# castorini/daam

Measured on NVIDIA H100. Metric: heatmap px/s (layers x steps x tokens), higher is better.
Workload: dtype bf16

## Files before the change

daam_b200/csrc/accumulate_mma.cu:

```cuda
#include <cuda.h>

#include <mutex>
#include <type_traits>
#include <unordered_map>
#include <string>

#include "common.cuh"

namespace daam {
namespace {

constexpr int kStages = 2;
constexpr int kAccStages = 3;
constexpr int kPrefetchTiles = 6;
constexpr int kQBytes = kTilePixels * 128;
constexpr int kKBytes = kTokensPad * 128;
constexpr int kStageBytes = kQBytes + kKBytes;
constexpr int kPBytes = kTokens * kTilePixels * 4;
constexpr int kConsumers = 256;
constexpr int kThreads = kConsumers + 32;
constexpr int kThreads16 = kConsumers + 64;
constexpr int kBarBytes = 64;
constexpr int kBarBytes16 = 8 * 2 * (kStages + kAccStages);
constexpr int kSmemBytes = 1024 + kStages * kStageBytes + kAccStages * kPBytes + kBarBytes16;
constexpr int kSlabSmemBytes = kSmemBytes + kPBytes;
constexpr int kSplitStageBytes = 2 * kStageBytes;
constexpr int kSplitSmemBytes = 1024 + (kStages + 1) * kSplitStageBytes + kPBytes + kBarBytes;
static_assert(kSmemBytes <= 232448, "16-bit form exceeds the 227 KB shared-memory limit");
static_assert(kSplitSmemBytes <= 232448, "split form exceeds the 227 KB shared-memory limit");
static_assert(kSlabSmemBytes <= 232448, "16-bit second-slab form exceeds the 227 KB shared-memory limit");
constexpr int long_smem_bytes(int chunks) {
  return 1024 + kStages * (kQBytes + chunks * kKBytes) + kAccStages * kPBytes + kBarBytes16;
}
static_assert(long_smem_bytes(3) <= 232448, "16-bit long-context form exceeds the 227 KB shared-memory limit");

struct MmaParams {
  LaunchParams base;
  CUtensorMap qmap[kMaxLayersPerLaunch];
  CUtensorMap kmap[kMaxLayersPerLaunch];
  CUtensorMap amap[kMaxLayersPerLaunch];
};
struct MmaSlabParams : MmaParams {
  CUtensorMap smap[kMaxLayersPerLaunch];
  float* slab[kMaxLayersPerLaunch];
};
template <bool kSecond>
using MmaParamsT = std::conditional_t<kSecond, MmaSlabParams, MmaParams>;

__device__ __forceinline__ uint32_t smem_u32(const void* p) { return (uint32_t)__cvta_generic_to_shared(p); }

__device__ __forceinline__ void mbar_init(uint32_t bar, uint32_t count) {
  asm volatile("mbarrier.init.shared::cta.b64 [%0], %1;" ::"r"(bar), "r"(count));
}
__device__ __forceinline__ void mbar_arrive(uint32_t bar) {
  asm volatile("mbarrier.arrive.shared::cta.b64 _, [%0];" ::"r"(bar) : "memory");
}
__device__ __forceinline__ void mbar_expect_tx(uint32_t bar, uint32_t bytes) {
  asm volatile("mbarrier.arrive.expect_tx.shared::cta.b64 _, [%0], %1;" ::"r"(bar), "r"(bytes) : "memory");
}
__device__ __forceinline__ bool mbar_try(uint32_t bar, uint32_t parity) {
  uint32_t ok;
  asm volatile(
      "{\n"
      ".reg .pred p;\n"
      "mbarrier.try_wait.parity.shared::cta.b64 p, [%1], %2;\n"
      "selp.u32 %0, 1, 0, p;\n"
      "}"
      : "=r"(ok)
      : "r"(bar), "r"(parity)
      : "memory");
  return ok != 0;
}
#ifndef DAAM_MBAR_TIMEOUT_CYCLES
#define DAAM_MBAR_TIMEOUT_CYCLES 20000000000LL
#endif
__device__ __forceinline__ void mbar_wait(uint32_t bar, uint32_t parity) {
  if (mbar_try(bar, parity)) return;
#if DAAM_MBAR_TIMEOUT_CYCLES > 0
  const long long t0 = clock64();
  while (!mbar_try(bar, parity)) {
    if (clock64() - t0 > DAAM_MBAR_TIMEOUT_CYCLES) __trap();
  }
#else
  while (!mbar_try(bar, parity)) {}
#endif
}

__device__ __forceinline__ void tma_load_4d(const CUtensorMap* map, uint32_t bar, uint32_t dst, int c0, int c1, int c2,
                                            int c3) {
  asm volatile(
      "cp.async.bulk.tensor.4d.shared::cluster.global.mbarrier::complete_tx::bytes [%0], [%1, {%3, %4, %5, %6}], [%2];"
      ::"r"(dst), "l"(reinterpret_cast<uint64_t>(map)), "r"(bar), "r"(c0), "r"(c1), "r"(c2), "r"(c3)
      : "memory");
}
__device__ __forceinline__ void tma_store_2d(const CUtensorMap* map, uint32_t src, int c0, int c1) {
  asm volatile("cp.async.bulk.tensor.2d.global.shared::cta.bulk_group [%0, {%2, %3}], [%1];" ::"l"(
                   reinterpret_cast<uint64_t>(map)),
               "r"(src), "r"(c0), "r"(c1)
               : "memory");
}
__device__ __forceinline__ void tma_reduce_add_2d(const CUtensorMap* map, uint32_t src, int c0, int c1) {
  asm volatile("cp.reduce.async.bulk.tensor.2d.global.shared::cta.add.tile.bulk_group [%0, {%2, %3}], [%1];" ::"l"(
                   reinterpret_cast<uint64_t>(map)),
               "r"(src), "r"(c0), "r"(c1)
               : "memory");
}
__device__ __forceinline__ uint64_t l2_evict_last() {
  uint64_t p;
  asm volatile("createpolicy.fractional.L2::evict_last.b64 %0, 1.0;" : "=l"(p));
  return p;
}
__device__ __forceinline__ uint64_t l2_evict_first() {
  uint64_t p;
  asm volatile("createpolicy.fractional.L2::evict_first.b64 %0, 1.0;" : "=l"(p));
  return p;
}
__device__ __forceinline__ void tma_prefetch_4d(const CUtensorMap* map, int c0, int c1, int c2, int c3, uint64_t pol) {
  asm volatile("cp.async.bulk.prefetch.tensor.4d.L2.global.tile.L2::cache_hint [%0, {%1, %2, %3, %4}], %5;"
               ::"l"(reinterpret_cast<uint64_t>(map)), "r"(c0), "r"(c1), "r"(c2), "r"(c3), "l"(pol)
               : "memory");
}
__device__ __forceinline__ void tma_load_2d_hint(const CUtensorMap* map, uint32_t bar, uint32_t dst, int c0, int c1,
                                                 uint64_t pol) {
  asm volatile(
      "cp.async.bulk.tensor.2d.shared::cluster.global.mbarrier::complete_tx::bytes.L2::cache_hint [%0], [%1, {%3, %4}], "
      "[%2], %5;"
      ::"r"(dst), "l"(reinterpret_cast<uint64_t>(map)), "r"(bar), "r"(c0), "r"(c1), "l"(pol)
      : "memory");
}
__device__ __forceinline__ void tma_store_2d_hint(const CUtensorMap* map, uint32_t src, int c0, int c1, uint64_t pol) {
  asm volatile("cp.async.bulk.tensor.2d.global.shared::cta.bulk_group.L2::cache_hint [%0, {%2, %3}], [%1], %4;" ::"l"(
                   reinterpret_cast<uint64_t>(map)),
               "r"(src), "r"(c0), "r"(c1), "l"(pol)
               : "memory");
}
__device__ __forceinline__ void prefetch_tensormap(const CUtensorMap* map) {
  asm volatile("prefetch.tensormap [%0];" ::"l"(reinterpret_cast<uint64_t>(map)) : "memory");
}
__device__ __forceinline__ void bulk_commit() { asm volatile("cp.async.bulk.commit_group;" ::: "memory"); }
__device__ __forceinline__ void bulk_wait_read0() { asm volatile("cp.async.bulk.wait_group.read 0;" ::: "memory"); }
__device__ __forceinline__ void bulk_wait_read1() { asm volatile("cp.async.bulk.wait_group.read 1;" ::: "memory"); }
__device__ __forceinline__ void fence_proxy_async() { asm volatile("fence.proxy.async.shared::cta;" ::: "memory"); }
__device__ __forceinline__ void consumer_barrier() { asm volatile("bar.sync 1, %0;" ::"n"(kConsumers) : "memory"); }

__device__ __forceinline__ uint64_t wgmma_desc_sw128(uint32_t smem_addr) {
  return (uint64_t)((smem_addr & 0x3FFFFu) >> 4) | (1ull << 16)  |
         ((uint64_t)(1024 >> 4) << 32)  | (1ull << 62) ;
}

using Frag = float[40];

__device__ __forceinline__ void frag_fence(Frag& d) {
#pragma unroll
  for (int i = 0; i < 40; ++i) asm volatile("" : "+f"(d[i])::"memory");
}
__device__ __forceinline__ void wgmma_fence() { asm volatile("wgmma.fence.sync.aligned;" ::: "memory"); }
__device__ __forceinline__ void wgmma_commit() { asm volatile("wgmma.commit_group.sync.aligned;" ::: "memory"); }
__device__ __forceinline__ void wgmma_wait0() { asm volatile("wgmma.wait_group.sync.aligned 0;" ::: "memory"); }

#define DAAM_FRAG_OPERANDS                                                                                          \
  "+f"(d[0]), "+f"(d[1]), "+f"(d[2]), "+f"(d[3]), "+f"(d[4]), "+f"(d[5]), "+f"(d[6]), "+f"(d[7]), "+f"(d[8]),         \
      "+f"(d[9]), "+f"(d[10]), "+f"(d[11]), "+f"(d[12]), "+f"(d[13]), "+f"(d[14]), "+f"(d[15]), "+f"(d[16]),          \
      "+f"(d[17]), "+f"(d[18]), "+f"(d[19]), "+f"(d[20]), "+f"(d[21]), "+f"(d[22]), "+f"(d[23]), "+f"(d[24]),         \
      "+f"(d[25]), "+f"(d[26]), "+f"(d[27]), "+f"(d[28]), "+f"(d[29]), "+f"(d[30]), "+f"(d[31]), "+f"(d[32]),         \
      "+f"(d[33]), "+f"(d[34]), "+f"(d[35]), "+f"(d[36]), "+f"(d[37]), "+f"(d[38]), "+f"(d[39])
#define DAAM_FRAG_REGS                                                                                              \
  "{%0, %1, %2, %3, %4, %5, %6, %7, %8, %9, %10, %11, %12, %13, %14, %15, %16, %17, %18, %19, %20, %21, %22, %23, " \
  "%24, %25, %26, %27, %28, %29, %30, %31, %32, %33, %34, %35, %36, %37, %38, %39}"

template <bool kBf16>
__device__ __forceinline__ void wgmma_16bit(Frag& d, uint64_t adesc, uint64_t bdesc) {
  if constexpr (kBf16)
    asm volatile("wgmma.mma_async.sync.aligned.m64n80k16.f32.bf16.bf16 " DAAM_FRAG_REGS ", %40, %41, 1, 1, 1, 0, 0;"
                 : DAAM_FRAG_OPERANDS
                 : "l"(adesc), "l"(bdesc)
                 : "memory");
  else
    asm volatile("wgmma.mma_async.sync.aligned.m64n80k16.f32.f16.f16 " DAAM_FRAG_REGS ", %40, %41, 1, 1, 1, 0, 0;"
                 : DAAM_FRAG_OPERANDS
                 : "l"(adesc), "l"(bdesc)
                 : "memory");
}
__device__ __forceinline__ void wgmma_tf32(Frag& d, uint64_t adesc, uint64_t bdesc) {
  asm volatile("wgmma.mma_async.sync.aligned.m64n80k8.f32.tf32.tf32 " DAAM_FRAG_REGS ", %40, %41, 1, 1, 1;"
               : DAAM_FRAG_OPERANDS
               : "l"(adesc), "l"(bdesc)
               : "memory");
}

struct Tile {
  int li, prompt, head, pixel0;
};
__device__ __forceinline__ Tile decode_tile(const LaunchParams& P, int tile, int& li) {
  while (li + 1 < P.n_layers && tile >= P.layer[li + 1].tile_begin) ++li;
  const LayerParams& L = P.layer[li];
  const int local = tile - L.tile_begin;
  const int ptile = local % L.tiles_per_head;
  const int ph = local / L.tiles_per_head;
  Tile t;
  t.li = li;
  t.head = ph % L.heads;
  t.prompt = ph / L.heads;
  t.pixel0 = ptile * kTilePixels;
  return t;
}

__device__ __forceinline__ int tile_at_weight(const LaunchParams& P, long long w) {
  if (w >= P.total_weight) return P.total_tiles;
  int li = 0;
  while (li + 1 < P.n_layers && w >= P.layer[li + 1].weight_begin) ++li;
  const LayerParams& L = P.layer[li];
  return L.tile_begin + (int)((w - L.weight_begin + L.weight - 1) / L.weight);
}

__device__ __forceinline__ float rna_tf32(float x) {
  uint32_t r;
  asm("cvt.rna.tf32.f32 %0, %1;" : "=r"(r) : "f"(x));
  return __uint_as_float(r);
}
__device__ __forceinline__ float trunc_tf32(float x) { return __uint_as_float(__float_as_uint(x) & 0xffffe000u); }

__device__ __forceinline__ void split_region(uint8_t* raw, uint8_t* lo, int begin, int end, int ctid, int n_conv) {
  const int stride = n_conv * 16;
  for (int off = begin + ctid * 16; off < end; off += 4 * stride) {
    float4 x[4];
#pragma unroll
    for (int u = 0; u < 4; ++u)
      if (off + u * stride < end) x[u] = *reinterpret_cast<const float4*>(raw + off + u * stride);
#pragma unroll
    for (int u = 0; u < 4; ++u)
      if (off + u * stride < end) {
        float4 h, l;
        h.x = trunc_tf32(x[u].x); h.y = trunc_tf32(x[u].y); h.z = trunc_tf32(x[u].z); h.w = trunc_tf32(x[u].w);
        l.x = rna_tf32(x[u].x - h.x); l.y = rna_tf32(x[u].y - h.y);
        l.z = rna_tf32(x[u].z - h.z); l.w = rna_tf32(x[u].w - h.w);
        *reinterpret_cast<float4*>(raw + off + u * stride) = h;
        *reinterpret_cast<float4*>(lo + off + u * stride) = l;
      }
  }
}

template <bool kBf16>
__device__ __forceinline__ void wgmma_chunk_16bit(Frag& d, uint32_t a_src, uint32_t k_src) {
  wgmma_fence();
#pragma unroll
  for (int k = 0; k < 4; ++k) wgmma_16bit<kBf16>(d, wgmma_desc_sw128(a_src + 32 * k), wgmma_desc_sw128(k_src + 32 * k));
  wgmma_commit();
  wgmma_wait0();
}
template <bool kBf16, int kC>
__device__ __forceinline__ void wgmma_chunk_16bit_long(Frag (&d)[kC], uint32_t a_src, uint32_t k_src) {
  wgmma_fence();
#pragma unroll
  for (int c = 0; c < kC; ++c)
#pragma unroll
    for (int k = 0; k < 4; ++k)
      wgmma_16bit<kBf16>(d[c], wgmma_desc_sw128(a_src + 32 * k), wgmma_desc_sw128(k_src + c * kKBytes + 32 * k));
  wgmma_commit();
  wgmma_wait0();
}

__device__ __forceinline__ void griddep_wait() { asm volatile("griddepcontrol.wait;" ::: "memory"); }

template <bool kSplit, bool kChunked, int kSlab, int kC = 1>
__global__ void __launch_bounds__(kSplit ? kThreads : kThreads16, 1)
accumulate_mma_kernel(const __grid_constant__ MmaParamsT<kSlab != kSlabNone> MP) {
  static_assert(kC == 1 || (!kSplit && kSlab == kSlabNone), "long contexts: 16-bit form, plain slab mode only");
  constexpr bool kSecond = kSlab != kSlabNone;
  constexpr int kCtx = kC * kTokens;
  constexpr int kStageBytesT = kSplit ? kSplitStageBytes : kQBytes + kC * kKBytes;
  constexpr int kOperandBytes = (kSplit ? kStages + 1 : kStages) * kStageBytesT;
  constexpr int kPTiles = kSplit ? 1 : kAccStages + (kSecond ? 1 : 0);
  const LaunchParams& P = MP.base;
  extern __shared__ uint8_t smem_raw[];
  const uint32_t raw = smem_u32(smem_raw);
  const uint32_t base = (raw + 1023u) & ~1023u;
  uint8_t* gen = smem_raw + (base - raw);
  float* sP = reinterpret_cast<float*>(gen + kOperandBytes);
  const uint32_t sP_u32 = base + kOperandBytes;
  float* sS = sP + kAccStages * (kTokens * kTilePixels);
  const uint32_t sS_u32 = sP_u32 + kAccStages * kPBytes;
  const uint32_t bars = sP_u32 + kPTiles * kPBytes;
  const uint32_t full0 = bars, empty0 = bars + 8 * kStages;
  const uint32_t afull0 = bars + 16 * kStages, aempty0 = afull0 + 8 * kAccStages;

  const int warp = threadIdx.x >> 5, lane = threadIdx.x & 31;
  int first, count, stride = 1;
  if constexpr (!kChunked && !kSplit) {
    first = blockIdx.x;
    stride = gridDim.x;
    count = (P.total_tiles - (int)blockIdx.x + stride - 1) / stride;
  } else if constexpr (!kChunked) {
    const int per = P.total_tiles / gridDim.x, rem = P.total_tiles % gridDim.x;
    first = blockIdx.x * per + min((int)blockIdx.x, rem);
    count = per + ((int)blockIdx.x < rem ? 1 : 0);
  } else {
    first = tile_at_weight(P, (long long)P.total_weight * blockIdx.x / gridDim.x);
    count = tile_at_weight(P, (long long)P.total_weight * (blockIdx.x + 1) / gridDim.x) - first;
  }

  if (threadIdx.x == 0) {
#pragma unroll
    for (int s = 0; s < kStages; ++s) {
      mbar_init(full0 + 8 * s, 1);
      mbar_init(empty0 + 8 * s, kConsumers / 32);
    }
    if constexpr (!kSplit) {
#pragma unroll
      for (int s = 0; s < kAccStages; ++s) {
        mbar_init(afull0 + 8 * s, 1);
        mbar_init(aempty0 + 8 * s, 1);
      }
    }
    asm volatile("fence.mbarrier_init.release.cluster;" ::: "memory");
  }
  if (count > 0 && lane == 0 && (warp == (kSplit ? 0 : 9) || warp == 8)) {
    int li0 = 0;
    const Tile t0 = decode_tile(P, first, li0);
    if (warp != 8) {
      prefetch_tensormap(&MP.amap[t0.li]);
      if constexpr (kSecond) prefetch_tensormap(&MP.smap[t0.li]);
    } else {
      prefetch_tensormap(&MP.qmap[t0.li]);
      prefetch_tensormap(&MP.kmap[t0.li]);
    }
  }
  __syncthreads();
  if (!P.early_loads) griddep_wait();
  asm volatile("griddepcontrol.launch_dependents;" ::: "memory");

  if (warp == 9) {
    if constexpr (!kSplit) {
      if (lane == 0 && count > 0) {
        if (P.early_loads) griddep_wait();
        const uint64_t pol = l2_evict_first();
        int li = 0;
        for (int i = 0; i < count; ++i) {
          const Tile t = decode_tile(P, first + i * stride, li);
#pragma unroll
          for (int c = 0; c < kC; ++c) {
            const int n = i * kC + c;
            const int a = n % kAccStages;
            mbar_wait(aempty0 + 8 * a, ((uint32_t)(n / kAccStages) & 1u) ^ 1u);
            mbar_expect_tx(afull0 + 8 * a, kPBytes);
            tma_load_2d_hint(&MP.amap[t.li], afull0 + 8 * a, sP_u32 + a * kPBytes, t.pixel0,
                             (t.prompt * P.layer[t.li].heads + t.head) * kCtx + c * kTokens, pol);
          }
        }
      }
    }
  } else if (warp == 8) {
    if (lane == 0) {
      int li = 0, j = 0;
      for (int i = 0; i < count; ++i) {
        if (!kSplit && P.early_loads && i == (kChunked ? 1 : kStages)) {
          const uint64_t pol = l2_evict_last();
          const int end = min(count, i + kPrefetchTiles);
          int pli = 0;
          Tile prev = decode_tile(P, first + (i - 1) * stride, pli);
          for (int p = i; p < end; ++p) {
            const Tile u = decode_tile(P, first + p * stride, pli);
            const bool new_head = u.li != prev.li || u.prompt != prev.prompt || u.head != prev.head;
            const int nc = kChunked ? (P.layer[u.li].head_dim + 63) >> 6 : 1;
            for (int c = 0; c < nc; ++c) {
              tma_prefetch_4d(&MP.qmap[u.li], 64 * c, u.head, u.pixel0, u.prompt, pol);
              if (new_head)
#pragma unroll
                for (int kc = 0; kc < kC; ++kc) tma_prefetch_4d(&MP.kmap[u.li], 64 * c, u.head, kc * kTokens, u.prompt, pol);
            }
            prev = u;
          }
        }
        const Tile t = decode_tile(P, first + i * stride, li);
        const int n_chunks = kChunked ? (P.layer[t.li].head_dim + 63) >> 6 : 1;
        for (int c = 0; c < n_chunks; ++c, ++j) {
          const int s = j % kStages;
          const uint32_t ph = (uint32_t)(j / kStages) & 1u;
          mbar_wait(empty0 + 8 * s, ph ^ 1u);
          const uint32_t q_dst = base + s * kStageBytesT;
          if constexpr (kSplit) {
            const uint32_t k_dst = q_dst + 2 * kQBytes;
            mbar_expect_tx(full0 + 8 * s, kStageBytesT);
            tma_load_4d(&MP.qmap[t.li], full0 + 8 * s, q_dst, 64 * c, t.head, t.pixel0, t.prompt);
            tma_load_4d(&MP.kmap[t.li], full0 + 8 * s, k_dst, 64 * c, t.head, 0, t.prompt);
            tma_load_4d(&MP.qmap[t.li], full0 + 8 * s, q_dst + kQBytes, 64 * c + 32, t.head, t.pixel0, t.prompt);
            tma_load_4d(&MP.kmap[t.li], full0 + 8 * s, k_dst + kKBytes, 64 * c + 32, t.head, 0, t.prompt);
          } else {
            const uint32_t k_dst = q_dst + kQBytes;
            mbar_expect_tx(full0 + 8 * s, kStageBytesT);
            tma_load_4d(&MP.qmap[t.li], full0 + 8 * s, q_dst, 64 * c, t.head, t.pixel0, t.prompt);
#pragma unroll
            for (int kc = 0; kc < kC; ++kc)
              tma_load_4d(&MP.kmap[t.li], full0 + 8 * s, k_dst + kc * kKBytes, 64 * c, t.head, kc * kTokens, t.prompt);
          }
        }
      }
    }
  } else {
    const int tid = threadIdx.x;
    const int wg = warp >> 2;
    const int quad = lane & 3;
    const int r0 = wg * 64 + (warp & 3) * 16 + (lane >> 2);
    int li = 0, j = 0;
    bool issued = false;
    for (int i = 0; i < count; ++i) {
      const Tile t = decode_tile(P, first + i * stride, li);
      const LayerParams& L = P.layer[t.li];
      const int n_chunks = kChunked ? (L.head_dim + 63) >> 6 : 1;
      Frag dd[kC];
      Frag& d = dd[0];
#pragma unroll
      for (int kc = 0; kc < kC; ++kc)
#pragma unroll
        for (int e = 0; e < 40; ++e) dd[kc][e] = 0.f;
      for (int c = 0; c < n_chunks; ++c, ++j) {
        const int s = j % kStages;
        mbar_wait(full0 + 8 * s, (uint32_t)(j / kStages) & 1u);
        const uint32_t q_src = base + s * kStageBytesT;
#pragma unroll
        for (int kc = 0; kc < kC; ++kc) frag_fence(dd[kc]);
        if constexpr (kSplit) {
          uint8_t* stage = gen + s * kStageBytesT;
          uint8_t* lo = gen + kStages * kStageBytesT;
          consumer_barrier();
          split_region(stage, lo, 0, kSplitStageBytes, tid, kConsumers);
          fence_proxy_async();
          consumer_barrier();
          wgmma_fence();
          const uint32_t q_lo = base + kStages * kStageBytesT;
          const uint32_t qa[3] = {q_lo, q_src, q_src};
          const uint32_t kb[3] = {q_src + 2 * kQBytes, q_lo + 2 * kQBytes, q_src + 2 * kQBytes};
#pragma unroll
          for (int p = 0; p < 3; ++p)
#pragma unroll
            for (int k = 0; k < 8; ++k)
              wgmma_tf32(d, wgmma_desc_sw128(qa[p] + (k >> 2) * kQBytes + wg * 64 * 128 + 32 * (k & 3)),
                         wgmma_desc_sw128(kb[p] + (k >> 2) * kKBytes + 32 * (k & 3)));
          wgmma_commit();
          wgmma_wait0();
        } else {
          const uint32_t a_src = q_src + wg * 64 * 128, k_src = q_src + kQBytes;
          if constexpr (kC == 1) {
            if (L.dtype == DAAM_BF16)
              wgmma_chunk_16bit<true>(d, a_src, k_src);
            else
              wgmma_chunk_16bit<false>(d, a_src, k_src);
          } else {
            if (L.dtype == DAAM_BF16)
              wgmma_chunk_16bit_long<true, kC>(dd, a_src, k_src);
            else
              wgmma_chunk_16bit_long<false, kC>(dd, a_src, k_src);
          }
        }
#pragma unroll
        for (int kc = 0; kc < kC; ++kc) frag_fence(dd[kc]);
        __syncwarp();
        if (lane == 0) mbar_arrive(empty0 + 8 * s);
      }

      float m0 = d[0], m1 = d[2];
#pragma unroll
      for (int kc = 0; kc < kC; ++kc)
#pragma unroll
      for (int jj = 0; jj < 10; ++jj) {
        const bool l0 = jj < 9 || quad <= 2, l1 = jj < 9 || quad < 2;
        if (l0) { m0 = fmaxf(m0, dd[kc][4 * jj]); m1 = fmaxf(m1, dd[kc][4 * jj + 2]); }
        if (l1) { m0 = fmaxf(m0, dd[kc][4 * jj + 1]); m1 = fmaxf(m1, dd[kc][4 * jj + 3]); }
      }
      m0 = fmaxf(m0, __shfl_xor_sync(0xffffffffu, m0, 1));
      m0 = fmaxf(m0, __shfl_xor_sync(0xffffffffu, m0, 2));
      m1 = fmaxf(m1, __shfl_xor_sync(0xffffffffu, m1, 1));
      m1 = fmaxf(m1, __shfl_xor_sync(0xffffffffu, m1, 2));
      const float sc = L.scale_log2e, mc0 = m0 * sc, mc1 = m1 * sc;
      float sum0 = 0.f, sum1 = 0.f;
#pragma unroll
      for (int kc = 0; kc < kC; ++kc)
#pragma unroll
      for (int jj = 0; jj < 10; ++jj) {
        const bool l0 = jj < 9 || quad <= 2, l1 = jj < 9 || quad < 2;
        float* f = dd[kc];
        f[4 * jj] = l0 ? fast_exp2(fmaf(f[4 * jj], sc, -mc0)) : 0.f;
        f[4 * jj + 2] = l0 ? fast_exp2(fmaf(f[4 * jj + 2], sc, -mc1)) : 0.f;
        f[4 * jj + 1] = l1 ? fast_exp2(fmaf(f[4 * jj + 1], sc, -mc0)) : 0.f;
        f[4 * jj + 3] = l1 ? fast_exp2(fmaf(f[4 * jj + 3], sc, -mc1)) : 0.f;
        sum0 += f[4 * jj] + f[4 * jj + 1];
        sum1 += f[4 * jj + 2] + f[4 * jj + 3];
      }
      sum0 += __shfl_xor_sync(0xffffffffu, sum0, 1);
      sum0 += __shfl_xor_sync(0xffffffffu, sum0, 2);
      sum1 += __shfl_xor_sync(0xffffffffu, sum1, 1);
      sum1 += __shfl_xor_sync(0xffffffffu, sum1, 2);
      const float inv0 = 1.0f / sum0, inv1 = 1.0f / sum1;

      if constexpr (!kSplit) {
#pragma unroll
        for (int kc = 0; kc < kC; ++kc) {
        const int n = i * kC + kc;
        const int a = n % kAccStages;
        float* sA = sP + a * (kTokens * kTilePixels);
        const bool lowq = quad < 2;
        const int ra = lowq ? r0 : r0 + 8, rb = lowq ? r0 + 8 : r0;
        mbar_wait(afull0 + 8 * a, (uint32_t)(n / kAccStages) & 1u);
        float old[40];
#pragma unroll
        for (int jj = 0; jj < 10; ++jj) {
#pragma unroll
          for (int e = 0; e < 2; ++e) {
            const int col = 8 * jj + 2 * quad + e;
            if (col < kTokens) {
              old[4 * jj + e] = sA[col * kTilePixels + ra];
              old[4 * jj + 2 + e] = sA[col * kTilePixels + rb];
            }
          }
        }
        if constexpr (kSecond) {
          if (tid == 0 && i > 0) bulk_wait_read0();
          consumer_barrier();
        }
        const float* f = dd[kc];
#pragma unroll
        for (int jj = 0; jj < 10; ++jj) {
#pragma unroll
          for (int e = 0; e < 2; ++e) {
            const int col = 8 * jj + 2 * quad + e;
            if (col < kTokens) {
              const float pa = f[4 * jj + e] * inv0, pb = f[4 * jj + 2 + e] * inv1;
              sA[col * kTilePixels + ra] = add_ftz(old[4 * jj + e], lowq ? pa : pb);
              sA[col * kTilePixels + rb] = add_ftz(old[4 * jj + 2 + e], lowq ? pb : pa);
              if constexpr (kSecond) {
                sS[col * kTilePixels + ra] = add_ftz(0.f, lowq ? pa : pb);
                sS[col * kTilePixels + rb] = add_ftz(0.f, lowq ? pb : pa);
              }
            }
          }
        }
        fence_proxy_async();
        consumer_barrier();
        if (tid == 0) {
          tma_store_2d_hint(&MP.amap[t.li], sP_u32 + a * kPBytes, t.pixel0,
                            (t.prompt * L.heads + t.head) * kCtx + kc * kTokens, l2_evict_first());
          if constexpr (kSlab == kSlabStore)
            tma_store_2d(&MP.smap[t.li], sS_u32, t.pixel0, (t.prompt * L.heads + t.head) * kTokens);
          if constexpr (kSlab == kSlabAdd)
            tma_reduce_add_2d(&MP.smap[t.li], sS_u32, t.pixel0, (t.prompt * L.heads + t.head) * kTokens);
          bulk_commit();
          if (n > 0) {
            bulk_wait_read1();
            mbar_arrive(aempty0 + 8 * ((n - 1) % kAccStages));
          }
        }
        }
        continue;
      }

      if (i == 0 && P.early_loads) griddep_wait();

      if (tid == 0 && issued) bulk_wait_read0();
      consumer_barrier();
      const bool lowq = quad < 2;
      const bool stage_ftz = kSlab == kSlabStore && P.rmw_mode == 1;
#pragma unroll
      for (int jj = 0; jj < 10; ++jj) {
#pragma unroll
        for (int e = 0; e < 2; ++e) {
          const int col = 8 * jj + 2 * quad + e;
          if (col < kTokens) {
            float a = d[4 * jj + e] * inv0, b = d[4 * jj + 2 + e] * inv1;
            if constexpr (kSecond) {
              if (stage_ftz) { a = add_ftz(0.f, a); b = add_ftz(0.f, b); }
            }
            sP[col * kTilePixels + (lowq ? r0 : r0 + 8)] = lowq ? a : b;
            sP[col * kTilePixels + (lowq ? r0 + 8 : r0)] = lowq ? b : a;
          }
        }
      }
      if (P.rmw_mode == 1) {
        fence_proxy_async();
        consumer_barrier();
        if (tid == 0) {
          tma_reduce_add_2d(&MP.amap[t.li], sP_u32, t.pixel0, (t.prompt * L.heads + t.head) * kTokens);
          if constexpr (kSlab == kSlabStore)
            tma_store_2d(&MP.smap[t.li], sP_u32, t.pixel0, (t.prompt * L.heads + t.head) * kTokens);
          if constexpr (kSlab == kSlabAdd)
            tma_reduce_add_2d(&MP.smap[t.li], sP_u32, t.pixel0, (t.prompt * L.heads + t.head) * kTokens);
          bulk_commit();
        }
        issued = true;
      } else {
        consumer_barrier();
        const long long hw = L.hw;
        float* acc = L.acc + ((long long)(t.prompt * L.heads + t.head) * kTokens) * hw + t.pixel0;
        const int live = min(kTilePixels, L.hw - t.pixel0) >> 2;
        for (int u = tid; u < kTokens * (kTilePixels / 4); u += kConsumers) {
          const int tok = u / (kTilePixels / 4), c4 = u % (kTilePixels / 4);
          if (c4 < live) {
            float4* g = reinterpret_cast<float4*>(acc + tok * hw) + c4;
            const float4 p = reinterpret_cast<const float4*>(sP + tok * kTilePixels)[c4];
            float4 o = *g;
            o.x += p.x; o.y += p.y; o.z += p.z; o.w += p.w;
            *g = o;
            if constexpr (kSlab == kSlabStore)
              reinterpret_cast<float4*>(MP.slab[t.li] + (acc - L.acc) + tok * hw)[c4] = p;
            if constexpr (kSlab == kSlabAdd) {
              float4* r = reinterpret_cast<float4*>(MP.slab[t.li] + (acc - L.acc) + tok * hw) + c4;
              float4 ro = *r;
              ro.x += p.x; ro.y += p.y; ro.z += p.z; ro.w += p.w;
              *r = ro;
            }
          }
        }
      }
    }
    if (tid == 0 && (kSplit ? issued : count > 0)) bulk_wait_read0();
  }
}

using EncodeFn = CUresult (*)(CUtensorMap*, CUtensorMapDataType, cuuint32_t, void*, const cuuint64_t*,
                              const cuuint64_t*, const cuuint32_t*, const cuuint32_t*, CUtensorMapInterleave,
                              CUtensorMapSwizzle, CUtensorMapL2promotion, CUtensorMapFloatOOBfill);

EncodeFn get_encode() {
  static EncodeFn fn = nullptr;
  static std::once_flag once;
  std::call_once(once, [] {
    void* p = nullptr;
    cudaDriverEntryPointQueryResult q;
    if (cudaGetDriverEntryPoint("cuTensorMapEncodeTiled", &p, cudaEnableDefault, &q) == cudaSuccess &&
        q == cudaDriverEntryPointSuccess)
      fn = reinterpret_cast<EncodeFn>(p);
  });
  return fn;
}

struct MapKey {
  const void* ptr;
  long long s1, s2, s3;
  int d1, d2, d3, kind;
  bool operator==(const MapKey& o) const {
    return ptr == o.ptr && s1 == o.s1 && s2 == o.s2 && s3 == o.s3 && d1 == o.d1 && d2 == o.d2 && d3 == o.d3 &&
           kind == o.kind;
  }
};
struct MapKeyHash {
  size_t operator()(const MapKey& k) const {
    size_t h = reinterpret_cast<size_t>(k.ptr);
    auto mix = [&h](long long v) { h ^= (size_t)v + 0x9e3779b97f4a7c15ull + (h << 6) + (h >> 2); };
    mix(k.s1); mix(k.s2); mix(k.s3); mix(k.d1); mix(k.d2); mix(k.d3); mix(k.kind);
    return h;
  }
};

std::unordered_map<MapKey, CUtensorMap, MapKeyHash>& map_cache() {
  static std::unordered_map<MapKey, CUtensorMap, MapKeyHash> c;
  return c;
}
std::mutex g_map_mu;

int make_qk_map(const void* ptr, int dtype, int head_dim, int heads, int rows, int prompts, long long s_head,
                long long s_row, long long s_prompt, int box_rows, CUtensorMap* out) {
  MapKey key{ptr, s_head, s_row, s_prompt, heads, rows, prompts * 1024 + box_rows, (dtype << 4) | (head_dim << 8)};
  {
    std::lock_guard<std::mutex> lock(g_map_mu);
    auto it = map_cache().find(key);
    if (it != map_cache().end()) { *out = it->second; return DAAM_OK; }
  }
  EncodeFn enc = get_encode();
  if (!enc) { set_error("cuTensorMapEncodeTiled is not available from this driver"); return DAAM_E_CUDA; }
  const cuuint64_t es = dtype == DAAM_F32 ? 4 : 2;
  const cuuint64_t dims[4] = {(cuuint64_t)head_dim, (cuuint64_t)heads, (cuuint64_t)rows, (cuuint64_t)prompts};
  auto bytes = [es](long long s) { return (cuuint64_t)(s > 0 ? s : 8) * es; };
  const cuuint64_t strides[3] = {bytes(s_head), bytes(s_row), bytes(s_prompt)};
  const cuuint32_t box[4] = {(cuuint32_t)(128 / es), 1, (cuuint32_t)box_rows, 1};
  const cuuint32_t estr[4] = {1, 1, 1, 1};
  const CUtensorMapDataType type = dtype == DAAM_F32    ? CU_TENSOR_MAP_DATA_TYPE_FLOAT32
                                   : dtype == DAAM_BF16 ? CU_TENSOR_MAP_DATA_TYPE_BFLOAT16
                                                        : CU_TENSOR_MAP_DATA_TYPE_FLOAT16;
  CUresult r = enc(out, type, 4, const_cast<void*>(ptr), dims, strides, box, estr, CU_TENSOR_MAP_INTERLEAVE_NONE,
                   CU_TENSOR_MAP_SWIZZLE_128B, CU_TENSOR_MAP_L2_PROMOTION_L2_128B, CU_TENSOR_MAP_FLOAT_OOB_FILL_NONE);
  if (r != CUDA_SUCCESS) { set_error("cuTensorMapEncodeTiled(q/k) failed with CUresult %d", (int)r); return DAAM_E_CUDA; }
  std::lock_guard<std::mutex> lock(g_map_mu);
  if (map_cache().size() > 8192) map_cache().clear();
  map_cache()[key] = *out;
  return DAAM_OK;
}

int make_acc_map(float* acc, int hw, int rows, CUtensorMap* out) {
  MapKey key{acc, 0, 0, 0, hw, rows, 0, 1};
  {
    std::lock_guard<std::mutex> lock(g_map_mu);
    auto it = map_cache().find(key);
    if (it != map_cache().end()) { *out = it->second; return DAAM_OK; }
  }
  EncodeFn enc = get_encode();
  if (!enc) { set_error("cuTensorMapEncodeTiled is not available from this driver"); return DAAM_E_CUDA; }
  const cuuint64_t dims[2] = {(cuuint64_t)hw, (cuuint64_t)rows};
  const cuuint64_t strides[1] = {(cuuint64_t)hw * 4};
  const cuuint32_t box[2] = {(cuuint32_t)kTilePixels, (cuuint32_t)kTokens};
  const cuuint32_t estr[2] = {1, 1};
  CUresult r = enc(out, CU_TENSOR_MAP_DATA_TYPE_FLOAT32, 2, acc, dims, strides, box, estr,
                   CU_TENSOR_MAP_INTERLEAVE_NONE, CU_TENSOR_MAP_SWIZZLE_NONE, CU_TENSOR_MAP_L2_PROMOTION_L2_128B,
                   CU_TENSOR_MAP_FLOAT_OOB_FILL_NONE);
  if (r != CUDA_SUCCESS) { set_error("cuTensorMapEncodeTiled(acc) failed with CUresult %d", (int)r); return DAAM_E_CUDA; }
  std::lock_guard<std::mutex> lock(g_map_mu);
  if (map_cache().size() > 8192) map_cache().clear();
  map_cache()[key] = *out;
  return DAAM_OK;
}

struct MmaInstance {
  const void* fn;
  int smem;
};
const MmaInstance kMmaInstances[] = {
    {(const void*)accumulate_mma_kernel<false, false, kSlabNone>, kSmemBytes},
    {(const void*)accumulate_mma_kernel<true, false, kSlabNone>, kSplitSmemBytes},
    {(const void*)accumulate_mma_kernel<false, true, kSlabNone>, kSmemBytes},
    {(const void*)accumulate_mma_kernel<true, true, kSlabNone>, kSplitSmemBytes},
    {(const void*)accumulate_mma_kernel<false, false, kSlabStore>, kSlabSmemBytes},
    {(const void*)accumulate_mma_kernel<true, false, kSlabStore>, kSplitSmemBytes},
    {(const void*)accumulate_mma_kernel<false, true, kSlabStore>, kSlabSmemBytes},
    {(const void*)accumulate_mma_kernel<true, true, kSlabStore>, kSplitSmemBytes},
    {(const void*)accumulate_mma_kernel<false, false, kSlabAdd>, kSlabSmemBytes},
    {(const void*)accumulate_mma_kernel<true, false, kSlabAdd>, kSplitSmemBytes},
    {(const void*)accumulate_mma_kernel<false, true, kSlabAdd>, kSlabSmemBytes},
    {(const void*)accumulate_mma_kernel<true, true, kSlabAdd>, kSplitSmemBytes},
    {(const void*)accumulate_mma_kernel<false, false, kSlabNone, 2>, long_smem_bytes(2)},
    {(const void*)accumulate_mma_kernel<false, true, kSlabNone, 2>, long_smem_bytes(2)},
    {(const void*)accumulate_mma_kernel<false, false, kSlabNone, 3>, long_smem_bytes(3)},
    {(const void*)accumulate_mma_kernel<false, true, kSlabNone, 3>, long_smem_bytes(3)},
};
constexpr int kLongVariant0 = 12;

std::once_flag g_attr_once[64];

}

struct PreparedMma {
  MmaSlabParams mp;
  int grid, block, variant;
  bool second;
};
void* prepared_mma_new() { return new PreparedMma; }
void prepared_mma_delete(void* p) { delete static_cast<PreparedMma*>(p); }

bool mma_supported(const LayerParams& L) {
  const bool prompts_ok = L.n_prompts == 1 || (L.qs_prompt > 0 && L.ks_prompt > 0);
  return L.head_dim % 8 == 0 && L.head_dim <= DAAM_MAX_HEAD_DIM && L.vec_ok && L.qs_head > 0 && L.qs_pixel > 0 &&
         L.ks_head > 0 && L.ks_token > 0 && prompts_ok && L.hw % 4 == 0;
}

int prepare_accumulate_mma(const LaunchParams& p, const SecondSlabs* slabs, SlabMode mode, const DeviceInfo& dev,
                           void* out) {
  if (dev.cc_major != 9) { set_error("the wgmma kernel needs an sm_90 device (found sm_%d%d)", dev.cc_major, dev.cc_minor); return DAAM_E_UNSUPPORTED; }
  PreparedMma& pm = *static_cast<PreparedMma*>(out);
  MmaSlabParams& mp = pm.mp;
  mp.base = p;
  const bool split = p.n_layers > 0 && p.layer[0].dtype == DAAM_F32;
  const int ctx = p.n_layers > 0 ? p.layer[0].tokens : kTokens;
  if ((ctx != kTokens && ctx != 2 * kTokens && ctx != 3 * kTokens) || (ctx != kTokens && (split || slabs))) {
    set_error("the wgmma kernel takes %d-token contexts, or 154 / 231 tokens for 16-bit layers without a second slab "
              "(got %d)", kTokens, ctx);
    return DAAM_E_UNSUPPORTED;
  }
  bool chunked = false;
  for (int i = 0; i < p.n_layers; ++i) {
    const LayerParams& L = p.layer[i];
    if ((L.dtype == DAAM_F32) != split) { set_error("mixed fp32 / 16-bit layers in one wgmma pack"); return DAAM_E_INVALID; }
    if (L.tokens != ctx) { set_error("mixed context lengths in one wgmma pack"); return DAAM_E_INVALID; }
    if (int rc = make_qk_map(L.q, L.dtype, L.head_dim, L.heads, L.hw, L.n_prompts, L.qs_head, L.qs_pixel, L.qs_prompt, kTilePixels, &mp.qmap[i])) return rc;
    if (int rc = make_qk_map(L.k, L.dtype, L.head_dim, L.heads, ctx, L.n_prompts, L.ks_head, L.ks_token, L.ks_prompt, kTokensPad, &mp.kmap[i])) return rc;
    if (int rc = make_acc_map(L.acc, L.hw, L.n_prompts * L.heads * ctx, &mp.amap[i])) return rc;
    if (slabs) {
      if (int rc = make_acc_map(slabs->slab[i], L.hw, L.n_prompts * L.heads * kTokens, &mp.smap[i])) return rc;
      mp.slab[i] = slabs->slab[i];
    }
    chunked = chunked || L.head_dim > 64;
  }
  cudaError_t attr_err = cudaSuccess;
  std::call_once(g_attr_once[dev.device & 63], [&] {
    for (const MmaInstance& k : kMmaInstances)
      if (cudaError_t e = cudaFuncSetAttribute(k.fn, cudaFuncAttributeMaxDynamicSharedMemorySize, k.smem)) attr_err = e;
  });
  DAAM_CUDA_TRY(attr_err);
  pm.grid = dev.sm_count;
  if (pm.grid > p.total_tiles) pm.grid = p.total_tiles;
  pm.block = split ? kThreads : kThreads16;
  pm.variant = ctx == kTokens ? (split ? 1 : 0) | (chunked ? 2 : 0) | (mode << 2)
                              : kLongVariant0 + (chunked ? 1 : 0) + (ctx == 3 * kTokens ? 2 : 0);
  pm.second = mode != kSlabNone;
  return DAAM_OK;
}

int launch_prepared_mma(const void* prepared, cudaStream_t stream) {
  const PreparedMma& pm = *static_cast<const PreparedMma*>(prepared);
  const MmaInstance& k = kMmaInstances[pm.variant];
  cudaLaunchConfig_t cfg = {};
  cfg.gridDim = dim3(pm.grid);
  cfg.blockDim = dim3(pm.block);
  cfg.dynamicSmemBytes = k.smem;
  cfg.stream = stream;
  cudaLaunchAttribute attr[1];
  attr[0].id = cudaLaunchAttributeProgrammaticStreamSerialization;
  attr[0].val.programmaticStreamSerializationAllowed = pm.mp.base.pdl ? 1 : 0;
  cfg.attrs = attr;
  cfg.numAttrs = 1;
  const MmaParams* plain = &pm.mp;
  void* args[] = {pm.second ? (void*)&pm.mp : (void*)plain};
  DAAM_CUDA_TRY(cudaLaunchKernelExC(&cfg, k.fn, args));
  DAAM_CUDA_TRY(cudaGetLastError());
  count_launch();
  return DAAM_OK;
}

}
```

Before: 268.1 billion.

## Move accumulator TMA stores to producer warp and add fourth accumulator slot

Consumer warps no longer synchronise on a named barrier and wait for the TMA store. Each warp now arrives on a per-slot 'done' mbarrier, and the producer warp issues the TMA store, waits for it to be read, and then reloads that slot. The plain 16-bit path gets a fourth accumulator slot, so loads and stores have more buffering ahead of the consumers. The second-slab case adds an sfree barrier that gates reuse of the slab staging tile. This takes store issue and the full consumer barrier off the consumers' critical path, at the cost of serialising store-then-load on one producer thread and using more shared memory.

```diff
diff --git a/daam_b200/csrc/accumulate_mma.cu b/daam_b200/csrc/accumulate_mma.cu
--- a/daam_b200/csrc/accumulate_mma.cu
+++ b/daam_b200/csrc/accumulate_mma.cu
@@ -11,7 +11,6 @@
 namespace {
 
 constexpr int kStages = 2;
-constexpr int kAccStages = 3;
 constexpr int kPrefetchTiles = 6;
 constexpr int kQBytes = kTilePixels * 128;
 constexpr int kKBytes = kTokensPad * 128;
@@ -21,18 +20,26 @@
 constexpr int kThreads = kConsumers + 32;
 constexpr int kThreads16 = kConsumers + 64;
 constexpr int kBarBytes = 64;
-constexpr int kBarBytes16 = 8 * 2 * (kStages + kAccStages);
-constexpr int kSmemBytes = 1024 + kStages * kStageBytes + kAccStages * kPBytes + kBarBytes16;
-constexpr int kSlabSmemBytes = kSmemBytes + kPBytes;
+__host__ __device__ constexpr int acc_slots(int slab, int chunks) {
+  return slab == kSlabNone && chunks == 1 ? 4 : 3;
+}
+constexpr int bar_bytes16(int slab, int chunks) {
+  return 8 * (2 * kStages + 2 * acc_slots(slab, chunks) + (slab != kSlabNone ? 1 : 0));
+}
+constexpr int smem16_bytes(int slab, int chunks) {
+  const int blocks = acc_slots(slab, chunks) + (slab != kSlabNone ? 1 : 0);
+  return 1024 + kStages * (kQBytes + chunks * kKBytes) + blocks * kPBytes + bar_bytes16(slab, chunks);
+}
+constexpr int kSmemBytes = smem16_bytes(kSlabNone, 1);
+constexpr int kSlabSmemBytes = smem16_bytes(kSlabStore, 1);
+constexpr int long_smem_bytes(int chunks) { return smem16_bytes(kSlabNone, chunks); }
 constexpr int kSplitStageBytes = 2 * kStageBytes;
 constexpr int kSplitSmemBytes = 1024 + (kStages + 1) * kSplitStageBytes + kPBytes + kBarBytes;
 static_assert(kSmemBytes <= 232448, "16-bit form exceeds the 227 KB shared-memory limit");
 static_assert(kSplitSmemBytes <= 232448, "split form exceeds the 227 KB shared-memory limit");
 static_assert(kSlabSmemBytes <= 232448, "16-bit second-slab form exceeds the 227 KB shared-memory limit");
-constexpr int long_smem_bytes(int chunks) {
-  return 1024 + kStages * (kQBytes + chunks * kKBytes) + kAccStages * kPBytes + kBarBytes16;
-}
-static_assert(long_smem_bytes(3) <= 232448, "16-bit long-context form exceeds the 227 KB shared-memory limit");
+static_assert(long_smem_bytes(2) <= 232448 && long_smem_bytes(3) <= 232448,
+              "16-bit long-context form exceeds the 227 KB shared-memory limit");
 
 struct MmaParams {
   LaunchParams base;
@@ -139,7 +146,6 @@
 }
 __device__ __forceinline__ void bulk_commit() { asm volatile("cp.async.bulk.commit_group;" ::: "memory"); }
 __device__ __forceinline__ void bulk_wait_read0() { asm volatile("cp.async.bulk.wait_group.read 0;" ::: "memory"); }
-__device__ __forceinline__ void bulk_wait_read1() { asm volatile("cp.async.bulk.wait_group.read 1;" ::: "memory"); }
 __device__ __forceinline__ void fence_proxy_async() { asm volatile("fence.proxy.async.shared::cta;" ::: "memory"); }
 __device__ __forceinline__ void consumer_barrier() { asm volatile("bar.sync 1, %0;" ::"n"(kConsumers) : "memory"); }
 
@@ -270,7 +276,8 @@
   constexpr int kCtx = kC * kTokens;
   constexpr int kStageBytesT = kSplit ? kSplitStageBytes : kQBytes + kC * kKBytes;
   constexpr int kOperandBytes = (kSplit ? kStages + 1 : kStages) * kStageBytesT;
-  constexpr int kPTiles = kSplit ? 1 : kAccStages + (kSecond ? 1 : 0);
+  constexpr int kSlots = acc_slots(kSlab, kC);
+  constexpr int kPTiles = kSplit ? 1 : kSlots + (kSecond ? 1 : 0);
   const LaunchParams& P = MP.base;
   extern __shared__ uint8_t smem_raw[];
   const uint32_t raw = smem_u32(smem_raw);
@@ -278,11 +285,11 @@
   uint8_t* gen = smem_raw + (base - raw);
   float* sP = reinterpret_cast<float*>(gen + kOperandBytes);
   const uint32_t sP_u32 = base + kOperandBytes;
-  float* sS = sP + kAccStages * (kTokens * kTilePixels);
-  const uint32_t sS_u32 = sP_u32 + kAccStages * kPBytes;
+  float* sS = sP + kSlots * (kTokens * kTilePixels);
+  const uint32_t sS_u32 = sP_u32 + kSlots * kPBytes;
   const uint32_t bars = sP_u32 + kPTiles * kPBytes;
   const uint32_t full0 = bars, empty0 = bars + 8 * kStages;
-  const uint32_t afull0 = bars + 16 * kStages, aempty0 = afull0 + 8 * kAccStages;
+  const uint32_t afull0 = bars + 16 * kStages, adone0 = afull0 + 8 * kSlots, sfree = adone0 + 8 * kSlots;
 
   const int warp = threadIdx.x >> 5, lane = threadIdx.x & 31;
   int first, count, stride = 1;
@@ -307,10 +314,11 @@
     }
     if constexpr (!kSplit) {
 #pragma unroll
-      for (int s = 0; s < kAccStages; ++s) {
+      for (int s = 0; s < kSlots; ++s) {
         mbar_init(afull0 + 8 * s, 1);
-        mbar_init(aempty0 + 8 * s, 1);
-      }
+        mbar_init(adone0 + 8 * s, kConsumers / 32);
+      }
+      if constexpr (kSecond) mbar_init(sfree, 1);
     }
     asm volatile("fence.mbarrier_init.release.cluster;" ::: "memory");
   }
@@ -334,18 +342,28 @@
       if (lane == 0 && count > 0) {
         if (P.early_loads) griddep_wait();
         const uint64_t pol = l2_evict_first();
-        int li = 0;
-        for (int i = 0; i < count; ++i) {
-          const Tile t = decode_tile(P, first + i * stride, li);
-#pragma unroll
-          for (int c = 0; c < kC; ++c) {
-            const int n = i * kC + c;
-            const int a = n % kAccStages;
-            mbar_wait(aempty0 + 8 * a, ((uint32_t)(n / kAccStages) & 1u) ^ 1u);
-            mbar_expect_tx(afull0 + 8 * a, kPBytes);
-            tma_load_2d_hint(&MP.amap[t.li], afull0 + 8 * a, sP_u32 + a * kPBytes, t.pixel0,
-                             (t.prompt * P.layer[t.li].heads + t.head) * kCtx + c * kTokens, pol);
-          }
+        const int total = count * kC;
+        int li_ld = 0, li_st = 0;
+        auto load = [&](int n) {
+          const Tile t = decode_tile(P, first + (n / kC) * stride, li_ld);
+          const int a = n % kSlots;
+          mbar_expect_tx(afull0 + 8 * a, kPBytes);
+          tma_load_2d_hint(&MP.amap[t.li], afull0 + 8 * a, sP_u32 + a * kPBytes, t.pixel0,
+                           (t.prompt * P.layer[t.li].heads + t.head) * kCtx + (n % kC) * kTokens, pol);
+        };
+        for (int n = 0; n < min(total, kSlots); ++n) load(n);
+        for (int n = 0; n < total; ++n) {
+          const int a = n % kSlots;
+          const Tile t = decode_tile(P, first + (n / kC) * stride, li_st);
+          const int row = t.prompt * P.layer[t.li].heads + t.head;
+          mbar_wait(adone0 + 8 * a, (uint32_t)(n / kSlots) & 1u);
+          tma_store_2d_hint(&MP.amap[t.li], sP_u32 + a * kPBytes, t.pixel0, row * kCtx + (n % kC) * kTokens, pol);
+          if constexpr (kSlab == kSlabStore) tma_store_2d(&MP.smap[t.li], sS_u32, t.pixel0, row * kTokens);
+          if constexpr (kSlab == kSlabAdd) tma_reduce_add_2d(&MP.smap[t.li], sS_u32, t.pixel0, row * kTokens);
+          bulk_commit();
+          bulk_wait_read0();
+          if constexpr (kSecond) mbar_arrive(sfree);
+          if (n + kSlots < total) load(n + kSlots);
         }
       }
     }
@@ -496,11 +514,11 @@
 #pragma unroll
         for (int kc = 0; kc < kC; ++kc) {
         const int n = i * kC + kc;
-        const int a = n % kAccStages;
+        const int a = n % kSlots;
         float* sA = sP + a * (kTokens * kTilePixels);
         const bool lowq = quad < 2;
         const int ra = lowq ? r0 : r0 + 8, rb = lowq ? r0 + 8 : r0;
-        mbar_wait(afull0 + 8 * a, (uint32_t)(n / kAccStages) & 1u);
+        mbar_wait(afull0 + 8 * a, (uint32_t)(n / kSlots) & 1u);
         float old[40];
 #pragma unroll
         for (int jj = 0; jj < 10; ++jj) {
@@ -514,8 +532,7 @@
           }
         }
         if constexpr (kSecond) {
-          if (tid == 0 && i > 0) bulk_wait_read0();
-          consumer_barrier();
+          if (i > 0) mbar_wait(sfree, (uint32_t)(i - 1) & 1u);
         }
         const float* f = dd[kc];
 #pragma unroll
@@ -535,20 +552,8 @@
           }
         }
         fence_proxy_async();
-        consumer_barrier();
-        if (tid == 0) {
-          tma_store_2d_hint(&MP.amap[t.li], sP_u32 + a * kPBytes, t.pixel0,
-                            (t.prompt * L.heads + t.head) * kCtx + kc * kTokens, l2_evict_first());
-          if constexpr (kSlab == kSlabStore)
-            tma_store_2d(&MP.smap[t.li], sS_u32, t.pixel0, (t.prompt * L.heads + t.head) * kTokens);
-          if constexpr (kSlab == kSlabAdd)
-            tma_reduce_add_2d(&MP.smap[t.li], sS_u32, t.pixel0, (t.prompt * L.heads + t.head) * kTokens);
-          bulk_commit();
-          if (n > 0) {
-            bulk_wait_read1();
-            mbar_arrive(aempty0 + 8 * ((n - 1) % kAccStages));
-          }
-        }
+        __syncwarp();
+        if (lane == 0) mbar_arrive(adone0 + 8 * a);
         }
         continue;
       }
@@ -611,7 +616,9 @@
         }
       }
     }
-    if (tid == 0 && (kSplit ? issued : count > 0)) bulk_wait_read0();
+    if constexpr (kSplit) {
+      if (tid == 0 && issued) bulk_wait_read0();
+    }
   }
 }
 
```

Result: no change. 270.6 billion (median of 6 runs) (+0.9%).
